# shenwei356/bio

Measured on AMD Instinct MI355X. Metric: Gbases/s hashed (k=21 ntHash + minimizer), higher is better.
Workload: dtype u64

## Files before the change

bio_amd/csrc/biosketch.hip:

```cpp
#include "host_internal.hpp"
#include "kernels_host.hpp"

extern "C" int bsk_abi_version(void) { return BSK_ABI_VERSION; }

extern "C" const char *bsk_err_name(int e) {
    switch (e) {
        case BSK_OK: return "ok";
        case BSK_ERR_INVALID_K: return "ErrInvalidK";
        case BSK_ERR_EMPTY_SEQ: return "ErrEmptySeq";
        case BSK_ERR_SHORT_SEQ: return "ErrShortSeq";
        case BSK_ERR_ILLEGAL_BASE: return "ErrIllegalBase";
        case BSK_ERR_K_TOO_LARGE: return "ErrKTooLarge";
        case BSK_ERR_INVALID_M: return "ErrInvalidM";
        case BSK_ERR_INVALID_SCALE: return "ErrInvalidScale";
        case BSK_ERR_INVALID_S: return "ErrInvalidS";
        case BSK_ERR_INVALID_W: return "ErrInvalidW";
        case BSK_ERR_BUF_NIL: return "ErrBufNil";
        case BSK_ERR_BUF_NOT_EMPTY: return "ErrBufNotEmpty";
        case BSK_ERR_ARG: return "bad argument";
        case BSK_ERR_NOMEM: return "out of memory";
        case BSK_ERR_DEVICE: return "device error";
        case BSK_ERR_UNSUPPORTED: return "unsupported";
        case BSK_ERR_NO_DEVICE: return "no gfx950 device";
        case BSK_ERR_IO: return "fastx: cannot open or read the file";
// ... 138 lines not shown

template <class LenOf>
static void collect_odd(bsk_batch *b, u64 n, LenOf len) {
    delete b->odd;
    b->odd = nullptr;
    b->modal_bucket = -1;
    if (!b->hist || n >= (1ULL << 32)) return;
    int mb = 0;
    for (int i = 1; i < LenHist::NB; ++i)
        if (b->hist->cnt[i] > b->hist->cnt[mb]) mb = i;
    const u64 others = n - b->hist->cnt[mb];
    if (others == 0 || others > n / 20) return;
    auto *v = new (std::nothrow) std::vector<u64>();
    if (!v) return;
    v->reserve((size_t)others);
    for (u64 r = 0; r < n; ++r) {
        const u64 L = len(r);
        if (LenHist::bucket(L) != mb) v->push_back((r << 32) | L);
    }
    b->odd = v;
    b->modal_bucket = mb;
}
static void upload_odd(bsk_ctx *ctx, bsk_batch *b) {
    (void)hipFree(b->d_odd);
    b->d_odd = nullptr;
    if (!b->odd || b->odd->size() < 65536) return;
    if (hipMalloc(&b->d_odd, b->odd->size() * sizeof(u64)) != hipSuccess) {
        (void)hipGetLastError();
        b->d_odd = nullptr;
        return;
    }
    if (hipMemcpyAsync(b->d_odd, b->odd->data(), b->odd->size() * sizeof(u64), hipMemcpyHostToDevice, ctx->stream) != hipSuccess) {
        (void)hipGetLastError();
        (void)hipFree(b->d_odd);
        b->d_odd = nullptr;
    }
}

u64 pad_words(u32 maxlen) { return (u64)maxlen / 16 + kMaxPrefetchWords + 1; }
u32 env_u32(const char *name, u32 dflt) {
    const char *v = getenv(name);
    return v && *v ? (u32)strtoul(v, nullptr, 10) : dflt;
}
u32 min_tile_min(const bsk_ctx *ctx) { return ctx->opt.tile_min ? ctx->opt.tile_min : std::min<u32>(64u, 16u * (BSK_NT_FAST_WORDS - 2)); }
void BskOpts::load() {
    auto on = [](const char *n) { return getenv(n) != nullptr; };
    force_generic = on("BSK_FORCE_GENERIC");
    no_mixed = on("BSK_NO_MIXED");
    no_dense = on("BSK_NO_DENSE");
    no_pk = on("BSK_NO_PK");
    no_ring = on("BSK_NO_RING");
    no_pkd = on("BSK_NO_PKD");
    no_side_early = on("BSK_NO_SIDE_EARLY");
    no_side_dense = on("BSK_NO_SIDE_DENSE");
    no_bin = on("BSK_NO_BIN");
    no_bin_early = on("BSK_NO_BIN_EARLY");
    compact = on("BSK_COMPACT");
    ring = on("BSK_RING");
    ring_max = env_u32("BSK_RING_MAX", 0);
    ring_sel10 = env_u32("BSK_RING_SEL10", 0);
    bin_min = env_u32("BSK_BIN_MIN", 1024);
    no_class = on("BSK_NO_CLASS");
    syn_sel = on("BSK_SYN_SEL");
    class_min = env_u32("BSK_CLASS_MIN", 16384);
    class_force = on("BSK_CLASS_FORCE");
    class_view = on("BSK_CLASS_VIEW");
    no_syn_pf = on("BSK_NO_SYN_PF");
    pf_density = env_u32("BSK_PF_DENSITY", 0);
    no_syn_long = on("BSK_NO_SYN_LONG");
    syn_margin = (int)env_u32("BSK_SYN_MARGIN", (u32)PlannerTable::syn_margin_rows + 64) - 64;
    no_tiles = on("BSK_NO_TILES");
    no_spare = on("BSK_NO_SPARE");
    no_tile_cache = on("BSK_NO_TILE_CACHE");
    tile_dense = on("BSK_TILE_DENSE");
    no_tile_defer = on("BSK_NO_TILE_DEFER");
    no_group_gather = on("BSK_NO_GROUP_GATHER");
    timing = on("BSK_TIMING");
    no_fused_translate = on("BSK_NO_FUSED_TRANSLATE");
    sets_no_small = on("BSK_SETS_NO_SMALL");
    wpr = env_u32("BSK_WPR", 0);
    seg = env_u32("BSK_SEG", 0);
    dense_min = env_u32("BSK_DENSE_MIN", (u32)PlannerTable::dense_min);
    waves_per_cu = env_u32("BSK_WAVES_PER_CU", 0);
    tile_min = env_u32("BSK_TILE_MIN", 0);
    tile_pos = env_u32("BSK_TILE_POS", 0);
    test_overflow = env_u32("BSK_TEST_OVERFLOW", 0);
}
extern "C" int bsk_build_has_experiments(void) {
#ifdef BSK_EXPERIMENTS
    return 1;
#else
    return 0;
#endif
}
extern "C" int bsk_ctx_reload_options(bsk_ctx *ctx) {
    if (!ctx) return BSK_ERR_ARG;
    ctx->opt.load();
    if (ctx->side) ctx->side->opt = ctx->opt;
    return BSK_OK;
}
bsk_ctx *side_ctx(bsk_ctx *ctx) {
    if (!ctx->side) {
        bsk_ctx *s = nullptr;
        if (bsk_ctx_create(ctx->device, &s) != BSK_OK) return nullptr;
        if (hipEventCreateWithFlags(&ctx->ev_side_done, hipEventDisableTiming) != hipSuccess || hipEventCreateWithFlags(&ctx->ev_adopted, hipEventDisableTiming) != hipSuccess ||
            hipEventCreateWithFlags(&ctx->ev_mix0, hipEventDisableTiming) != hipSuccess || hipEventCreateWithFlags(&ctx->ev_mix1, hipEventDisableTiming) != hipSuccess ||
            hipEventCreateWithFlags(&ctx->ev_tiled, hipEventDisableTiming) != hipSuccess) {
            bsk_ctx_destroy(s);
            return nullptr;
        }
        ctx->side = s;
    }
    ctx->side->opt = ctx->opt;
    return ctx->side;
}

static int batch_from_ascii_impl(bsk_ctx *ctx, const uint8_t *bytes, const uint64_t *offsets, uint64_t n, int alphabet, bsk_batch *donor,
                                 bsk_batch **out) {
    if (!ctx || !out || (!offsets && n) || (n && !bytes && offsets[n] > 0)) return fail_arg(ctx, "bsk_batch_from_ascii: null argument");
    if (alphabet < BSK_ALPHA_DNA || alphabet > BSK_ALPHA_UNLIMIT) return fail_arg(ctx, "bad alphabet");
    const int pairs = alphabet == BSK_ALPHA_PROTEIN ? BSK_ALPHA_DNA : alphabet;
    if (alphabet != BSK_ALPHA_PROTEIN) alphabet = BSK_ALPHA_DNA;
    *out = nullptr;
    HIPCHK(ctx, hipSetDevice(ctx->device));
    if (donor && !donor->ascii && donor->spare_ascii) {
        donor->ascii = donor->spare_ascii;
        donor->aoff = donor->spare_aoff;
        donor->spare_ascii = nullptr;
        donor->spare_aoff = nullptr;
    }
    auto take = [&](void **dst, size_t *cap_dst, size_t need, void **src, size_t *cap_src) -> hipError_t {
        if (donor && src && *src && *cap_src >= need) {
            *dst = *src;
            *cap_dst = *cap_src;
            *src = nullptr;
            *cap_src = 0;
            return hipSuccess;
        }
        const size_t want = donor ? need + need / 8 + 256 : need;
        const hipError_t e = hipMalloc(dst, want ? want : 1);
        if (e == hipSuccess) *cap_dst = want;
        return e;
    };
    struct DonorGuard {
        bsk_batch *d;
        ~DonorGuard() { if (d) bsk_batch_destroy(d); }
    } donor_guard{donor};
    bsk_batch *b = new (std::nothrow) bsk_batch();
    if (!b) return BSK_ERR_NOMEM;
    b->ctx = ctx;
    b->alphabet = alphabet;
    b->pairs = pairs;
    b->n = n;
    if (donor) {
        std::swap(b->bdesc, donor->bdesc);
        std::swap(b->c_bdesc, donor->c_bdesc);
        std::swap(b->bflags, donor->bflags);
        std::swap(b->c_bflags, donor->c_bflags);
    }
    const u64 nbytes = n ? offsets[n] : 0;
    b->n_bases = nbytes;
    u32 maxlen = 0;
    bool uniform = true;
    for (u64 r = 0; r < n; ++r) {
        if (offsets[r + 1] < offsets[r]) {
            delete b;
// ... 996 lines not shown
```

bio_amd/csrc/host_types.hpp:

```cpp
#pragma once
#include <hip/hip_runtime.h>

#include <cstdio>
#include <string>
#include <vector>

#include "biosketch.h"
#include "device_common.hpp"

struct BskOpts {
    bool force_generic = false, no_mixed = false, no_dense = false, no_pk = false, no_ring = false, no_pkd = false, no_side_early = false, no_side_dense = false, ring = false, no_bin = false, no_bin_early = false, compact = false, no_spare = false, no_tiles = false, no_tile_cache = false, no_tile_defer = false, tile_dense = false, no_group_gather = false, timing = false,
         no_fused_translate = false, sets_no_small = false;
    int syn_margin = 2;
    u32 test_overflow = 0;
    bool no_syn_long = false;
    u32 pf_density = 0;
    bool no_syn_pf = false;
    bool syn_sel = false;
    bool no_class = false;
    u32 class_min = 16384;
    bool class_view = false;
    bool class_force = false;
    u32 wpr = 0, seg = 0, dense_min = 21 , ring_max = 0, ring_sel10 = 0 , bin_min = 1024, waves_per_cu = 0, tile_min = 0, tile_pos = 0;
    void load();
};

struct bsk_ctx {
    BskOpts opt;
    int device = 0;
    int cus = 0;
    hipStream_t stream = nullptr;
    std::string err;
    u32 *d_ticket = nullptr;
    u64 *d_total = nullptr;
    u64 *d_lookback = nullptr;
    size_t lookback_cap = 0;
    u64 *d_ring_h = nullptr;
    u32 *d_ring_p = nullptr;
    size_t ring_cap = 0;
    u64 *h_pinned = nullptr;
    u8 *d_lut = nullptr;
    int lut_table = 0;
    void *tmp[32] = {};
    size_t tmp_cap[32] = {};
    u64 *h_refs = nullptr;
    size_t h_refs_cap = 0;
    struct bsk_result *tile_res = nullptr;
    static constexpr int SPARE_SLOTS = 8;
    struct Spare {
        void *p = nullptr;
        size_t bytes = 0;
    } spare[SPARE_SLOTS];
    size_t spare_bytes = 0, spare_limit = 0;
    void *comm = nullptr;
    int comm_rank = 0, comm_world = 0;
    u64 *d_comm = nullptr;
    bsk_ctx *side = nullptr;
    hipEvent_t ev_side_done = nullptr, ev_adopted = nullptr, ev_mix0 = nullptr, ev_mix1 = nullptr, ev_tiled = nullptr;
    bool adopted_recorded = false;
    struct ClassSet *cls = nullptr;
    bool no_side_fast = false;
    struct bsk_result *cls_owner = nullptr;
    u64 sel_need = 0;
    bool no_syn_pk = false;
    bool no_prot_fast = false;
    bool defer = false;
    bool tile_sync = false;
    bool tile_async = false;
    bool tile_was_async = false;
    bool in_resize = false;
    int cls_round = 0;
    bool part_grow = false;
    bool no_dense = false;
};

struct LenHist {
    static constexpr int NB = 160;
    u64 cnt[NB] = {}, bases[NB] = {};
    u32 hi[NB] = {};
    u32 lo[NB];
    LenHist() {
        for (int i = 0; i < NB; ++i) lo[i] = 0xffffffffu;
    }
    static int bucket(u64 L) {
        if (L < 1024) return (int)(L >> 4);
        const int lg = 63 - __builtin_clzll(L);
        return 64 + 4 * (lg - 10) + (int)((L >> (lg - 2)) & 3);
    }
    void add(u64 L) {
        const int i = bucket(L);
        cnt[i]++;
        bases[i] += L;
        if ((u32)L > hi[i]) hi[i] = (u32)L;
        if ((u32)L < lo[i]) lo[i] = (u32)L;
    }
};

struct bsk_batch {
    bsk_ctx *ctx = nullptr;
    int alphabet = BSK_ALPHA_DNA;
    int pairs = BSK_ALPHA_DNA;
    u64 n = 0, n_bases = 0, n_words = 0, n_nonacgt = 0;
    u32 maxlen = 0;
    u32 side_maxlen = 0;
    u32 uniform_len = 0;
    u32 *words = nullptr;
// ... 85 lines not shown
```

bio_amd/csrc/kernels_pk.hpp:

```cpp
#pragma once
#include <utility>

#include "kernels_fast.hpp"

namespace bsk {

template <int... Is, class F>
__device__ __forceinline__ void pk_unroll_impl(std::integer_sequence<int, Is...>, F &&f) {
    (f(std::integral_constant<int, Is>{}), ...);
}
template <int N, class F>
__device__ __forceinline__ void pk_unroll(F &&f) {
    pk_unroll_impl(std::make_integer_sequence<int, N>{}, f);
}

#ifndef BSK_PK_ROWS
#define BSK_PK_ROWS 58
#endif
struct PkLds {
    static constexpr int PR = BSK_PK_ROWS;
    static constexpr int ROW = 33;
    static constexpr int TAB = 0;
    static constexpr int TAB2 = 320;
    static constexpr int NHEADS = (32 * (PR - 1)) / 64 + 2;
    static constexpr int HEADS = 0;
    static constexpr int CTAB = 256;
    static constexpr int SH = 768;
    static constexpr int SP = SH + (PR + 1) * ROW * 8;
    static constexpr int TOTAL = (SP + (PR + 1) * ROW * 2 + 15) & ~15;
    static_assert(NHEADS * 8 <= CTAB && CTAB + 512 <= SH && TAB2 + 256 <= SH && TOTAL <= 20480, "PkLds");
};

struct PkTabs {
    u32x4 row;
    u32 at;
    __device__ __forceinline__ void init(int k, int lane, u32 tab = (u32)PkLds::TAB, u32 tab2 = (u32)PkLds::TAB2) {
        row = (u32x4){0, 0, 0, 0};
        at = 0xffffffffu;
        if (lane < 20) {
            const unsigned out = (unsigned)lane >> 2, in = (unsigned)lane & 3u;
            u64 f = seed_fwd_code(in);
            u64 r = rol64(seed_rev_code(in), (unsigned)(k - 1));
            if (out < 4) {
                f ^= rol64(seed_fwd_code(out), (unsigned)k);
                r ^= ror64(seed_rev_code(out), 1);
            }
            row = (u32x4){(u32)f, (u32)(f >> 32), (u32)r, (u32)(r >> 32)};
            at = tab + (u32)lane * 16u;
        } else if (lane >= 32 && lane < 48) {
            const unsigned c0 = (unsigned)lane & 3u, c1 = ((unsigned)lane >> 2) & 3u;
            const u64 f = rol64(seed_fwd_code(c0), 1) ^ seed_fwd_code(c1);
            const u64 r = ror64(rol64(seed_rev_code(c0), (unsigned)(k - 1)), 1) ^ rol64(seed_rev_code(c1), (unsigned)(k - 1));
            row = (u32x4){(u32)f, (u32)(f >> 32), (u32)r, (u32)(r >> 32)};
            at = tab2 + (u32)(lane - 32) * 16u;
        }
    }
    __device__ __forceinline__ void write(LDSQ char *ldsq) const {
        if (at != 0xffffffffu) *reinterpret_cast<LDSQ u32x4 *>(ldsq + at) = row;
        wave_sync_lds();
    }
};

template <int W>
struct PkCfg {
    static constexpr int XC = W > 12 ? 4 : W;
};

#define PKNW 16
typedef u32 u32x16 __attribute__((ext_vector_type(16)));
struct PkWords {
    u32x4 a, b, c, d;
};
__device__ __forceinline__ PkWords pk_load_words(const u32 *p) {
    PkWords r;
    asm volatile("global_load_dwordx4 %0, %4, off\n\tglobal_load_dwordx4 %1, %4, off offset:16\n\t"
                 "global_load_dwordx4 %2, %4, off offset:32\n\tglobal_load_dwordx4 %3, %4, off offset:48"
                 : "=&v"(r.a), "=&v"(r.b), "=&v"(r.c), "=&v"(r.d)
                 : "v"(p));
    return r;
}
__device__ __forceinline__ u64 pk_load_u64(const u64 *p) {
    u64 r;
    asm volatile("global_load_dwordx2 %0, %1, off" : "=&v"(r) : "v"(p));
    return r;
}
__device__ __forceinline__ void pk_wait_loads(u64 &d0, u64 &d1) { asm volatile("s_waitcnt vmcnt(0)" : "+v"(d0), "+v"(d1)::"memory"); }
__device__ __forceinline__ void pk_wait_loads(PkWords &p) { asm volatile("s_waitcnt vmcnt(0)" : "+v"(p.a), "+v"(p.b), "+v"(p.c), "+v"(p.d)::"memory"); }
__device__ __forceinline__ void pk_ticket_async(u32 *ticket, u32 &t) {
    u64 ex;
    asm volatile("s_mov_b64 %1, exec\n\ts_mov_b64 exec, 1\n\tglobal_atomic_add %0, %2, %3, off sc0\n\ts_mov_b64 exec, %1"
                 : "+v"(t), "=&s"(ex)
                 : "v"(ticket), "v"(1u)
                 : "memory");
}
__device__ __forceinline__ void pk_wait_loads(PkWords &p, u64 &d0, u32 &f, u32 &t) {
    asm volatile("s_waitcnt vmcnt(0)" : "+v"(p.a), "+v"(p.b), "+v"(p.c), "+v"(p.d), "+v"(d0), "+v"(f), "+v"(t)::"memory");
}
__device__ __forceinline__ u32 pk_load_u8(const u8 *p) {
    u32 r;
    asm volatile("global_load_ubyte %0, %1, off" : "=&v"(r) : "v"(p));
    return r;
}
template <int W, bool LONG, class LY_ = PkLds, bool RINGM = false, bool SELM = false>
struct PkMin {
    typedef LY_ LY;
    const u32 *__restrict__ w;
    LDSQ char *lds;
    int k, lane;
    u32 nk;
    u32 fl, fh_, rl, rh_;
    u32 S[W];
    u64 H[W];
    u32 SB[W];
    u32 P, bm, tmin;
    u32 nsel;
    u32 slot, spare;
    u32 glo, gspan;
    u32 c8000;
    int sstep;
    u32 send;
    u32 in_lo, in_hi, out_lo, out_hi;
    u32x4 pw;
    u32x16 wr;
    static constexpr bool POS2 = !RINGM && !SELM;
    u32 i2;

    __device__ __forceinline__ void set_words(const PkWords &p) {
        wr = (u32x16){p.a.x, p.a.y, p.a.z, p.a.w, p.b.x, p.b.y, p.b.z, p.b.w, p.c.x, p.c.y, p.c.z, p.c.w, p.d.x, p.d.y, p.d.z, p.d.w};
    }
    __device__ __forceinline__ void word2(u32 i, u32 &lo, u32 &hi) const {
        const u32 iu = (u32)__builtin_amdgcn_readfirstlane((int)i);
        if (!LONG || iu + 1 < (u32)PKNW) {
            lo = wr[iu], hi = wr[iu + 1];
        } else {
            lo = w[iu], hi = w[iu + 1];
        }
    }
    __device__ __forceinline__ u32 word(u32 i) const {
        const u32 iu = (u32)__builtin_amdgcn_readfirstlane((int)i);
        if constexpr (RINGM) {
            if (iu < 4u) return iu == 0 ? pw.x : iu == 1 ? pw.y : iu == 2 ? pw.z : pw.w;
            return w[iu];
        }
        if (!LONG || iu < (u32)PKNW) return wr[iu];
        return w[iu];
    }
    __device__ __forceinline__ void load_block_words(u32 i0) {
        const u32 t0 = i0 + (u32)k - 1, p0 = i0 - 1;
        in_lo = w[t0 >> 4];
        in_hi = w[(t0 >> 4) + 1];
        out_lo = w[p0 >> 4];
        out_hi = w[(p0 >> 4) + 1];
// ... 119 lines not shown
            const u32 nv = (u32)(left < 0 ? 0 : left > W ? W : left);
            vb = (1u << nv) - 1u;
        }
        pk_unroll<W>([&](auto oc) {
            constexpr int o = decltype(oc)::value;
            if (XC < W && o && o % XC == 0 && o + XC < W) {
                __builtin_amdgcn_sched_barrier(0);
                fetch(o + XC);
            }
            roll(xs[o]);
            if (!FIRST) this->template emit<PB + o, o>(pbase);
            const lmask rev = lt64(rl, rh_, fl, fh_);
            const u32 hl = sel(rev, rl, fl), hh = sel(rev, rh_, fh_);
            if constexpr (POS2) {
                lmask co;
                asm("v_addc_co_u32_e64 %0, %1, %2, %3, %4" : "=v"(SB[o]), "=s"(co) : "n"(2 * o), "v"(i2), "s"(rev));
            } else {
                asm("v_cndmask_b32_e64 %0, 0, %1, %2" : "=v"(SB[o]) : "v"(c8000), "s"(rev));
            }
            H[o] = ((u64)hh << 32) | hl;
            u32 pk;
            asm("v_and_or_b32 %0, %1, %2, %3" : "=v"(pk) : "v"(hh), "s"(0xffffffe0u), "n"(CB + o));
            if (o == 0) {
                P = pk;
            } else {
#ifndef PK_NOTIE
                const u32 d = pk ^ P;
                tmin = tmin < d ? tmin : d;
#endif
                P = P < pk ? P : pk;
            }
            if (!FIRST || o == W - 1) {
                u32 m = P;
                if constexpr (o != W - 1) {
#ifndef PK_NOTIE
                    const u32 d = P ^ S[o + 1];
                    tmin = tmin < d ? tmin : d;
#endif
                    m = P < S[o + 1] ? P : S[o + 1];
                }
                u32 one = 1u;
                if (FIRST) one = okbit;
                else if (RAG) one = (vb >> o) & 1u;
                bm |= one << (m & 31u);
            }
            S[o] = pk;
        });
        if (suffix) {
#pragma unroll
            for (int q = W - 2; q >= 0; --q) {
#ifndef PK_NOTIE
                const u32 d = S[q] ^ S[q + 1];
                tmin = tmin < d ? tmin : d;
#endif
                S[q] = S[q] < S[q + 1] ? S[q] : S[q + 1];
            }
        }
        if constexpr (SELM) {
            if (!FIRST) {
                const u32 wsel = (bm >> PB) & ((1u << W) - 1u);
                *reinterpret_cast<LDSQ u32 *>(lds + LY::MASK + (i0 / (u32)W - 1u) * 256u + (u32)lane * 4u) = wsel;
                nsel += (u32)__builtin_popcount(wsel);
            }
        }
        if (!FIRST) bm &= PAR ? 0xffff0000u : 0x0000ffffu;
    }

    template <int PAR>
    __device__ __forceinline__ void drain(u32 i0) {
        if constexpr (SELM) {
            const u32 wsel = (bm >> (PAR * 16)) & ((1u << W) - 1u);
            *reinterpret_cast<LDSQ u32 *>(lds + LY::MASK + (i0 / (u32)W) * 256u + (u32)lane * 4u) = wsel;
            nsel += (u32)__builtin_popcount(wsel);
            return;
        }
        const u32 pbase = (u32)__builtin_amdgcn_readfirstlane((int)i0);
        guard();
        pk_unroll<W>([&](auto oc) {
            constexpr int o = decltype(oc)::value;
            this->template emit<PAR * 16 + o, o>(pbase);
        });
    }

    __device__ __forceinline__ void begin(u32 slot0, int step, u32 col8) {
        fl = fh_ = rl = rh_ = 0;
        bm = 0;
        nsel = 0;
        c8000 = 0x8000u;
        asm volatile("" : "+v"(c8000));
        tmin = 0xffffffffu;
        slot = slot0;
        sstep = step;
        if constexpr (RINGM) {
            (void)col8;
            spare = glo = gspan = 0;
            send = (u32)(LY::ROWS * LY::ROW * 8) + (u32)lane * 8u;
        } else {
            spare = (u32)(LY::PR * LY::ROW * 8) + col8;
            send = 0;
            constexpr u32 RB = (u32)(LY::ROW * 8);
            glo = step < 0 ? col8 + (u32)(W - 1) * RB : col8;
            gspan = (u32)(LY::PR - W) * RB + (step < 0 ? 0u : RB);
        }
        if constexpr (RINGM) load_block0_words();
        for (int t0 = 0; t0 < k - 1; t0 += 16) {
            const u32 word = this->word((u32)t0 >> 4);
            const int nb = (k - 1 - t0) < 16 ? (k - 1 - t0) : 16;
            int j = 0;
            for (; j + 8 <= nb; j += 8) {
                const u32 sub = word >> (2 * j);
                const u32x4 x0 = *reinterpret_cast<LDSQ const u32x4 *>(lds + LY::TAB2 + ((sub & 0xf) << 4));
                const u32x4 x1 = *reinterpret_cast<LDSQ const u32x4 *>(lds + LY::TAB2 + (sub & 0xf0));
                const u32x4 x2 = *reinterpret_cast<LDSQ const u32x4 *>(lds + LY::TAB2 + ((sub & 0xf00) >> 4));
                const u32x4 x3 = *reinterpret_cast<LDSQ const u32x4 *>(lds + LY::TAB2 + ((sub & 0xf000) >> 8));
                roll2(x0);
                roll2(x1);
                roll2(x2);
                roll2(x3);
            }
            for (; j + 2 <= nb; j += 2) roll2(*reinterpret_cast<LDSQ const u32x4 *>(lds + LY::TAB2 + (((word >> (2 * j)) & 0xf) << 4)));
            for (; j < nb; ++j) roll(*reinterpret_cast<LDSQ const u32x4 *>(lds + LY::TAB + 256 + (((word >> (2 * j)) & 3) << 4)));
        }
    }

    __device__ __forceinline__ void run(u32 nk_max, bool ok, u32 nk_min, u32 slot0, int step, u32 col8) {
        begin(slot0, step, col8);
        block<true, false, 0>(0, ok ? 1u : 0u, nk_max > (u32)W);
        u32 i0 = W;
        int last_par = 0;
        for (;;) {
            if (i0 >= nk_max) break;
            {
                const bool more = i0 + W < nk_max;
                if (i0 + W <= nk_min) block<false, false, 1>(i0, 1u, more);
                else block<false, true, 1>(i0, 1u, more);
            }
            i0 += W;
            last_par = 1;
            if (i0 >= nk_max) break;
            {
                const bool more = i0 + W < nk_max;
                if (i0 + W <= nk_min) block<false, false, 0>(i0, 1u, more);
                else block<false, true, 0>(i0, 1u, more);
            }
            i0 += W;
            last_par = 0;
        }
        if (last_par) drain<1>(i0 - W);
        else drain<0>(i0 - W);
    }
};

template <int U, class LY = PkLds, bool POS2 = false>
__device__ __forceinline__ void pk_copyout(char *lds, int lane, u32 cnt, u32 excl, u32 T, u64 base, const KArgs &a) {
    constexpr int NH = LY::NHEADS;
    u64 *s_heads = reinterpret_cast<u64 *>(lds + LY::HEADS);
    u64 *s_tab64 = reinterpret_cast<u64 *>(lds + LY::CTAB);
    const u64 nzmask = __builtin_amdgcn_ballot_w64(cnt > 0);
    if (lane < NH) s_heads[lane] = 0;
    wave_sync_lds();
    if (cnt > 0) {
        constexpr int RB = LY::ROW * 8;
        const int col8 = (lane & 31) * 8;
        const int S = lane < 32 ? RB : -RB;
        const int A = lane < 32 ? col8 - (int)excl * RB : col8 + ((int)(LY::PR - 1) + (int)excl) * RB;
        const u32 rk = __builtin_amdgcn_mbcnt_hi((u32)(nzmask >> 32), __builtin_amdgcn_mbcnt_lo((u32)nzmask, 0));
        s_tab64[rk] = ((u64)(u32)S << 32) | (u32)A;
        if (excl) atomicOr(&s_heads[(excl - 1u) >> 6], 1ULL << ((excl - 1u) & 63u));
    }
    wave_sync_lds();
    const u64 hw = lane < NH ? s_heads[lane] : 0ULL;
    const u32 hw_lo = (u32)hw, hw_hi = (u32)(hw >> 32);
    u32 heads_before = 0;
    const char *sh = lds + LY::SH, *sp = lds + LY::SP;
    u64 *const gh = a.hash + base;
    u32 *const gp = a.pos + base;
    auto trip = [&](u32 t0, auto check) {
        constexpr bool CHECK = decltype(check)::value;
        u32 rank[U];
#pragma unroll
        for (int j = 0; j < U; ++j) {
            const u32 c = (t0 >> 6) + j;
            const u32 mlo = (u32)__builtin_amdgcn_readlane((int)hw_lo, (int)c), mhi = (u32)__builtin_amdgcn_readlane((int)hw_hi, (int)c);
            rank[j] = (__builtin_amdgcn_mbcnt_hi(mhi, __builtin_amdgcn_mbcnt_lo(mlo, 0u)) << 3) + (heads_before << 3);
            heads_before += (u32)__builtin_popcountll(((u64)mhi << 32) | mlo);
        }
        u64 ent[U];
#pragma unroll
        for (int j = 0; j < U; ++j) ent[j] = *reinterpret_cast<const u64 *>(reinterpret_cast<const char *>(s_tab64) + rank[j]);
        if constexpr (U == 8) {
            __builtin_amdgcn_sched_barrier(0);
            asm volatile("" ::"v"(ent[0]), "v"(ent[1]), "v"(ent[2]), "v"(ent[3]), "v"(ent[4]), "v"(ent[5]), "v"(ent[6]), "v"(ent[7]));
            __builtin_amdgcn_sched_barrier(0);
        }
        u64 hv[U];
        u32 pv[U];
#pragma unroll
        for (int j = 0; j < U; ++j) {
            const u32 t = t0 + 64 * j + lane;
            const int off = __mul24((int)t, (int)(u32)(ent[j] >> 32)) + (int)(u32)ent[j];
            const u32 so = (!CHECK || t < T) ? (u32)off : 0u;
            hv[j] = *reinterpret_cast<const u64 *>(sh + so);
            if constexpr (POS2) pv[j] = *reinterpret_cast<const u16 *>(sp + (so >> 2));
            else pv[j] = (u32)(int)*reinterpret_cast<const short *>(sp + (so >> 2));
        }
        if constexpr (U == 8) {
            __builtin_amdgcn_sched_barrier(0);
            asm volatile("" ::"v"(hv[0]), "v"(hv[1]), "v"(hv[2]), "v"(hv[3]), "v"(hv[4]), "v"(hv[5]), "v"(hv[6]), "v"(hv[7]), "v"(pv[0]), "v"(pv[1]),
                         "v"(pv[2]), "v"(pv[3]), "v"(pv[4]), "v"(pv[5]), "v"(pv[6]), "v"(pv[7]));
            __builtin_amdgcn_sched_barrier(0);
        }
#pragma unroll
        for (int j = 0; j < U; ++j) {
            const u32 t = t0 + 64 * j + lane;
#ifdef PK_NOSTORE
            asm volatile("" ::"v"(hv[j]), "v"(pv[j]));
#else
            if (!CHECK || t < T) {
#ifndef PK_NOHASHST
                __builtin_nontemporal_store(hv[j], &gh[t]);
#else
                asm volatile("" ::"v"(hv[j]));
#endif
#ifndef PK_NOPOSST
                __builtin_nontemporal_store(POS2 ? __builtin_amdgcn_alignbit(pv[j], pv[j], 1) : pv[j] & 0x80007fffu, &gp[t]);
#else
                asm volatile("" ::"v"(pv[j]));
#endif
            }
#endif
        }
    };
    u32 t0 = 0;
    for (; t0 + 64 * U <= T; t0 += 64 * U) trip(t0, std::false_type{});
    if (t0 < T) trip(t0, std::true_type{});
    wave_sync_lds();
}

#ifndef PK_TICKET
#define PK_TICKET 8u
#endif
template <int W, bool LONG>
__global__ __launch_bounds__(64, 2) void k_minimizer_pk(KArgs a) {
    typedef PkLds LY;
    __shared__ __attribute__((aligned(16))) char lds[LY::TOTAL];
    LDSQ char *const ldsq = (LDSQ char *)lds;
    const int lane = lane_id();
    PkTabs tabs;
    tabs.init(a.k, lane);
#ifdef PK_STAGGER
    for (u32 i = (((blockIdx.x * 2654435761u) >> 24) * (u32)PK_STAGGER) >> 8; i; --i) __builtin_amdgcn_s_sleep(32);
#endif
    const u64 slab = (u64)64 * BSK_FAST_CAP;
    const u32 col8 = (u32)(lane & 31) * 8u;
    constexpr u32 RB = (u32)(LY::ROW * 8);
    const u32 top = (u32)(LY::PR - 1) * RB + col8;
    u64 d_n1 = 0, d_cur = 0;
    PkWords pw_cur = {{0, 0, 0, 0}, {0, 0, 0, 0}, {0, 0, 0, 0}, {0, 0, 0, 0}};
    bool have = false;
    const u32 lseg = a.fixcap / a.list_grid;
    u32 lcur = 0;
    const u32 tku = a.tk ? a.tk : PK_TICKET;
    const bool ahead = tku >= 3u;
    u32 tv = 0;
    u32 nt = ~0u;
    for (u32 unit = next_ticket(a.ticket, lane) * tku, uend = unit + tku; unit < a.nunits; ++unit, ({
             if (unit == uend) {
                 unit = ahead ? nt : next_ticket(a.ticket, lane) * tku;
                 uend = unit + tku;
             }
         })) {
        const u64 r = (u64)unit * 64 + lane;
        const u64 u2 = (!ahead || unit + 2u < uend) ? (u64)unit + 2u : (u64)nt + (unit + 2u - uend);
        const bool nxt = unit + 1 != uend ? unit + 1 < a.nunits : ahead && nt < a.nunits;
        const bool ask = ahead && unit + 3u == uend;
        const u64 rmax = a.n - 1;
        if (!have) {
            d_cur = pk_load_u64(a.desc + (r < rmax ? r : rmax));
            d_n1 = pk_load_u64(a.desc + (r + 64 < rmax ? r + 64 : rmax));
            pk_wait_loads(d_cur, d_n1);
            pw_cur = pk_load_words(a.words + (d_cur >> 24));
            pk_wait_loads(pw_cur);
        }
        PkWords pw_n1 = pk_load_words(a.words + (d_n1 >> 24));
        const u64 r2 = u2 * 64 + lane;
        u64 d_n2 = pk_load_u64(a.desc + (r2 < rmax ? r2 : rmax));
        u32 rfl = pk_load_u8(a.rflags ? a.rflags + (r < rmax ? r : rmax) : reinterpret_cast<const u8 *>(a.desc));
        if (ask) pk_ticket_async(a.ticket, tv);
        const u64 d = d_cur;
        const PkWords pw = pw_cur;
        const u64 off = d >> 24, L = desc_len(a, d);
        const u64 ro = out_index(a, r, d);
        const bool ok = r < a.n && L >= (u64)a.circ_ext && (L - (u64)a.circ_ext) + 1 >= (u64)a.k + (u64)W;
        const u32 nk = ok ? (u32)(L - a.k + 1) : 0u;
        const u32 nk_max = wave_max_u32(nk);
        const u32 nk_min = ~wave_max_u32(~(ok ? nk : 0xffffffffu));
        u32 cnt = 0, tmin_lane = 0xffffffffu;
        if (nk_max) {
            tabs.write(ldsq);
            PkMin<W, LONG> pm;
            pm.w = a.words + off;
            pm.set_words(pw);
            pm.lds = ldsq;
            pm.k = a.k;
            pm.lane = lane;
            pm.nk = nk;
            const u32 spare = (u32)LY::PR * RB + col8;
            pm.run(nk_max, ok, nk_min, !ok ? spare : lane < 32 ? col8 : top, !ok ? 0 : lane < 32 ? (int)RB : -(int)RB, col8);
            if (ok) cnt = (lane < 32 ? pm.slot - col8 : top - pm.slot) / RB;
            tmin_lane = pm.tmin;
        }
        pk_wait_loads(pw_n1, d_n2, rfl, tv);
        if (ask) nt = (u32)__builtin_amdgcn_readfirstlane((int)tv) * tku;
        d_cur = d_n1;
        pw_cur = pw_n1;
        d_n1 = d_n2;
        have = nxt;
        const u32 cnt_pair = cnt + (u32)__builtin_amdgcn_ds_bpermute((lane ^ 32) * 4, (int)cnt);
        u64 bad = __builtin_amdgcn_ballot_w64(cnt_pair >= (u32)LY::PR);
        u64 tied = __builtin_amdgcn_ballot_w64(ok && tmin_lane < 32u);
#if defined(PK_NOSTAGE) || defined(PK_NOTIE) || defined(PK_NOTAB) || defined(PK_NOCOPY) || defined(PK_NOSTORE) || defined(PK_NOFB)
        bad = 0;
        tied = 0;
#endif
        const u64 redo = bad | tied;
        if (redo) {
            list_append(a, a.rlist, lseg, lcur, redo, lane, r);
            if ((redo >> lane) & 1) cnt = 0;
        }
        const u32 incl = wave_incl_scan_u32(cnt, lane);
        const u32 excl = incl - cnt;
        const u32 T = wave_bcast_u32(incl, 63);
        const u64 base = (u64)unit * slab;
#ifndef PK_NOCOPY
#ifndef PK_CU
#define PK_CU 8
#endif
        if (T) pk_copyout<PK_CU, LY, PkMin<W, LONG>::POS2>(lds, lane, cnt, excl, T, base, a);
#endif
        if (r < a.n) {
            if (!((redo >> lane) & 1)) a.refs[ro] = ((base + excl) << 24) | cnt;
            u8 sbyte = ok ? BSK_ST_OK : BSK_ST_SHORT;
            if (ok && a.rflags) sbyte |= (u8)rfl;
            a.status[ro] = sbyte;
        }
    }
    list_close(a.rlist, lseg, lcur, lane);
}

#ifdef BSK_IMPL_PK
#ifndef BSK_PK_WS
#define BSK_PK_WS(X) X(2) X(3) X(4) X(5) X(6) X(7) X(8) X(9) X(10) X(11) X(12) X(13)
#endif
bool pk_minimizer_supported(int w) { return w >= 2 && w <= 13; }
u32 pk_minimizer_short_bases() { return 16u * (PKNW - 1); }
int pk_minimizer_blocks_per_cu(int w) {
    int nb = 0;
    hipError_t e = hipErrorInvalidValue;
    switch (w) {
#define X(WW) \
    case WW: e = hipOccupancyMaxActiveBlocksPerMultiprocessor(&nb, k_minimizer_pk<WW, false>, 64, 0); break;
        BSK_PK_WS(X)
#undef X
        default: break;
    }
    if (e != hipSuccess || nb < 1) {
        (void)hipGetLastError();
        nb = 1;
    }
    return nb;
}
void pk_minimizer_list_launch(int w, int grid, hipStream_t stream, const KArgs &a) {
    switch (w) {
#define X(WW) \
    case WW: hipLaunchKernelGGL((k_minimizer_dense<WW, true>), dim3(grid), dim3(64), 0, stream, a); break;
        BSK_PK_WS(X)
#undef X
        default: break;
    }
}
void pk_minimizer_launch(int w, bool long_reads, int grid, hipStream_t stream, const KArgs &a) {
    switch (w) {
#define X(WW)                                                                                               \
    case WW:                                                                                                \
        if (long_reads) {                                                                                   \
            hipLaunchKernelGGL((k_minimizer_pk<WW, true>), dim3(grid), dim3(64), 0, stream, a);             \
        } else {                                                                                            \
            hipLaunchKernelGGL((k_minimizer_pk<WW, false>), dim3(grid), dim3(64), 0, stream, a);            \
        }                                                                                                   \
        hipLaunchKernelGGL((k_minimizer_dense<WW, true>), dim3(grid), dim3(64), 0, stream, a);              \
        break;
        BSK_PK_WS(X)
#undef X
        default: break;
    }
// ... 5 lines not shown
```

bio_amd/csrc/planner.hip:

```cpp
#include "host_internal.hpp"
#include "kernels_host.hpp"

int validate(const bsk_params *p, int alphabet) {
    switch (p->kind) {
        case BSK_NTHASH:
            if (p->k < 1) return BSK_ERR_INVALID_K;
            break;
        case BSK_KMER:
            if (p->k < 1) return BSK_ERR_INVALID_K;
            if (p->k > 32) return BSK_ERR_K_TOO_LARGE;
            break;
        case BSK_SIMHASH:
            if (p->k < 1) return BSK_ERR_INVALID_K;
            if (p->k >= 65535) return BSK_ERR_K_TOO_LARGE;
            if (p->m < 4 || p->m > p->k) return BSK_ERR_INVALID_M;
            if (p->scale < 1 || p->scale > p->k - p->m + 1) return BSK_ERR_INVALID_SCALE;
            if (p->k - p->m + 1 > 32767) return BSK_ERR_UNSUPPORTED;
            break;
        case BSK_MINIMIZER:
            if (p->k < 1) return BSK_ERR_INVALID_K;
            if (p->w < 1) return BSK_ERR_INVALID_W;
            break;
        case BSK_SYNCMER:
            if (p->k < 1) return BSK_ERR_INVALID_K;
// ... 340 lines not shown
            pl.slab = true;
            pl.slab_unit = (u64)64 * BSK_SYN_CAP;
            pl.slab_total = (u64)pl.nunits * pl.slab_unit;
            pl.bin_gran = bin_gran_for(ctx, b, p->k - p->s);
            per_cu = fast_syncmer_blocks_per_cu(pl.fast_w);
        } else {
            pl.which = use_ascii ? K_SYN_A : K_SYN_P;
            per_cu = use_ascii ? occ(OCC_SYN_A) : occ(OCC_SYN_P);
            pl.ring_w = (u32)std::max(1, 2 * (p->k - p->s));
        }
    } else if (p->kind == BSK_KMER) {
        if (!use_ascii && p->canonical > 0 && b->maxlen + (u32)(p->circular ? p->k : 0) <= 16u * (BSK_NT_FAST_WORDS - 2) &&
            !ctx->opt.force_generic) {
            pl.which = K_NT_FAST;
            pl.compact = stream_compact_ok(ctx, b, p);
            per_cu = occ(OCC_NT_FAST2);
#ifdef BSK_EXPERIMENTS
            if (pl.compact) per_cu = occ(OCC_NT_FAST2C);
#endif
        } else if (!use_ascii && p->canonical <= 0 && !p->circular && b->maxlen <= 16u * (BSK_NT_FAST_WORDS - 2) && !ctx->opt.force_generic) {
            pl.which = K_NT_FAST;
            per_cu = occ(p->canonical < 0 ? OCC_NT_FAST4 : OCC_NT_FAST3);
        } else {
            pl.which = use_ascii ? K_KMER_A : K_KMER_P;
            per_cu = use_ascii ? occ(OCC_KMER_A) : occ(OCC_KMER_P);
        }
    } else if (p->kind == BSK_SIMHASH) {
        const int nh = p->k - p->m + 1;
        if (!use_ascii && nh <= 63 && b->maxlen + (u32)(p->circular ? p->k : 0) <= 16u * (BSK_NT_FAST_WORDS - 2) &&
            !ctx->opt.force_generic) {
            pl.which = K_SIM_FAST;
            pl.fast_w = nh <= 31 ? 5 : 6;
            const u32 ext_len = b->maxlen + (u32)(p->circular ? p->k : 0);
            pl.fast_k = ext_len <= 16u * (BSK_SIM_SHORT_WORDS - 2) ? 1 : ext_len <= 16u * (BSK_SIM_MID_WORDS - 2) ? 2 : 0;
            if (pl.fast_k == 1) per_cu = nh <= 31 ? occ(OCC_SIMF_5S) : occ(OCC_SIMF_6S);
            else if (pl.fast_k == 2) per_cu = nh <= 31 ? occ(OCC_SIMF_5M) : occ(OCC_SIMF_6M);
            else per_cu = nh <= 31 ? occ(OCC_SIMF_5) : occ(OCC_SIMF_6);
        } else {
            pl.which = use_ascii ? K_SIM_A : K_SIM_P;
            per_cu = use_ascii ? occ(OCC_SIM_A) : occ(OCC_SIM_P);
            pl.ring_w = (u32)nh;
        }
    } else if (p->kind == BSK_PROT_HASH) {
        if (b->alphabet == BSK_ALPHA_DNA) {
            pl.which = K_PROT_HASH_FAST;
            pl.fused_dna = true;
            pl.fast_k = p->k;
            per_cu = fast_prot_hash_dna_blocks_per_cu(p->k);
        } else if (fast_prot_hash_supported(p->k) && !ctx->opt.force_generic) {
            pl.which = K_PROT_HASH_FAST;
            pl.fast_k = p->k;
            per_cu = fast_prot_hash_blocks_per_cu(p->k);
        } else {
            pl.which = K_PROT_HASH;
            per_cu = occ(OCC_PROT_HASH);
        }
    } else if (p->kind == BSK_PROT_MINIMIZER) {
        const u32 plen = b->alphabet == BSK_ALPHA_DNA ? (u32)translated_len(b->maxlen, 1) : b->maxlen;
        if (b->alphabet == BSK_ALPHA_DNA && ctx->no_prot_fast) return BSK_REPLAN_UNFUSED;
        if (b->alphabet == BSK_ALPHA_DNA || (fast_prot_supported(p->w, p->k) && b->maxlen < 65536u && b->maxlen >= (u32)(p->k + p->w) && !ctx->opt.force_generic &&
            !ctx->no_prot_fast && slab_budget_ok(b, (u64)b->maxlen))) {
            pl.which = K_PROT_MIN_FAST;
            pl.fused_dna = b->alphabet == BSK_ALPHA_DNA;
            pl.fast_w = p->w;
            pl.fast_k = p->k;
            pl.slab = true;
            const u64 nwin = plen >= (u32)(p->k + p->w) ? (u64)plen - p->k - p->w + 2 : 1;
            pl.slab_read = std::min<u64>(nwin, (u64)(nwin * PlannerTable::slab_sel_num / (p->w + 1.0)) + PlannerTable::slab_sel_pad);
            pl.slab_read = (pl.slab_read + 15) & ~(u64)15;
            pl.slab_unit = 64 * pl.slab_read;
            pl.slab_total = (u64)pl.nunits * pl.slab_unit;
            per_cu = fast_prot_blocks_per_cu(p->w, p->k);
        } else {
            pl.which = K_PROT_MIN;
            per_cu = occ(OCC_PROT_MIN);
            pl.ring_w = (u32)p->w;
        }
    } else {
        ctx->err = "unknown kind";
        return BSK_ERR_ARG;
    }
    if (ctx->opt.waves_per_cu) per_cu = (int)ctx->opt.waves_per_cu;
    pl.grid = (int)std::max<u64>(1, std::min<u64>((u64)ctx->cus * per_cu, pl.nunits));
    pl.ring_entries = (size_t)pl.grid * pl.ring_w * 64;
    return BSK_OK;
}


void plan_name(const Plan &pl, const bsk_params *p, bool tiled, int cus, bsk_result *res) {
    char b[80];
    switch (pl.which) {
        case K_MIN_GEN_P: snprintf(b, sizeof b, "k_minimizer_generic<0>"); break;
        case K_MIN_GEN_A: snprintf(b, sizeof b, "k_minimizer_generic<1>"); break;
        case K_NT_P: snprintf(b, sizeof b, "k_nthash_stream<0>"); break;
        case K_NT_A: snprintf(b, sizeof b, "k_nthash_stream<1>"); break;
        case K_MIN_FAST: snprintf(b, sizeof b, "k_minimizer_fast<%d,%d,true>", pl.fast_w, BSK_FAST_CAP); break;
        case K_MIN_PK: snprintf(b, sizeof b, "k_minimizer_pk<%d,%s>", pl.fast_w, pl.fast_k ? "true" : "false"); break;
        case K_MIN_RING: snprintf(b, sizeof b, "k_minimizer_ring<%d,%s>", pl.fast_w, pl.fast_k ? "true" : "false"); break;
        case K_MIN_DENSE: snprintf(b, sizeof b, "k_minimizer_dense<%d>", pl.fast_w); break;
        case K_MIN_PKD: snprintf(b, sizeof b, "k_minimizer_pkd<%d>", pl.fast_w); break;
        case K_MIN_SEG: snprintf(b, sizeof b, "k_minimizer_seg<%d>", pl.fast_w); break;
        case K_MIN_WPR: snprintf(b, sizeof b, "k_minimizer_wpr<%d>", pl.fast_w); break;
        case K_NT_FAST: snprintf(b, sizeof b, pl.compact ? "k_nthash_fast<%d,true>" : "k_nthash_fast<%d>", p->kind == BSK_KMER ? (p->canonical > 0 ? 2 : p->canonical < 0 ? 4 : 3) : p->canonical ? 1 : 0); break;
        case K_SYN_P: snprintf(b, sizeof b, "k_syncmer<0>"); break;
        case K_SYN_A: snprintf(b, sizeof b, "k_syncmer<1>"); break;
        case K_KMER_P: snprintf(b, sizeof b, "k_kmer<0>"); break;
        case K_KMER_A: snprintf(b, sizeof b, "k_kmer<1>"); break;
        case K_SIM_P: snprintf(b, sizeof b, "k_simhash<0>"); break;
        case K_SIM_A: snprintf(b, sizeof b, "k_simhash<1>"); break;
        case K_PROT_HASH: snprintf(b, sizeof b, "k_prot_hash"); break;
        case K_PROT_MIN: snprintf(b, sizeof b, "k_prot_minimizer"); break;
        case K_SYN_FAST: snprintf(b, sizeof b, "k_syncmer_fast<%d>", pl.fast_w); break;
        case K_SYN_PK: snprintf(b, sizeof b, pl.syn_fused ? (pl.syn_long ? "k_syncmer_pfl<%d>" : "k_syncmer_pf<%d>") : pl.syn_long ? "k_syncmer_pkl<%d>" : "k_syncmer_pk<%d>", pl.fast_w); break;
        case K_SYN_SEL: snprintf(b, sizeof b, "k_syncmer_sel<%d> + k_syncmer_emit", pl.fast_w); break;
        case K_PROT_MIN_FAST: snprintf(b, sizeof b, "k_prot_minimizer_fast<%d,%d,%s>", pl.fast_w, pl.fast_k, pl.fused_dna ? "true" : "false"); break;
        case K_PROT_HASH_FAST: snprintf(b, sizeof b, "k_prot_hash_fast<%d,%s>", pl.fast_k, pl.fused_dna ? "true" : "false"); break;
        case K_SIM_FAST:
            snprintf(b, sizeof b, "k_simhash_fast<%d,%d>", pl.fast_w, pl.fast_k == 1 ? BSK_SIM_SHORT_WORDS : pl.fast_k == 2 ? BSK_SIM_MID_WORDS : BSK_NT_FAST_WORDS);
            break;
        default: snprintf(b, sizeof b, "?"); break;
    }
    snprintf(res->plan, sizeof res->plan, "%s%s%s%s", b, pl.bin_gran ? " (length-binned units)" : "", pl.mixed ? " + ASCII side launch" : "", tiled ? " (over tiles)" : "");
    res->plan_grid = pl.grid;
    res->plan_per_cu = cus > 0 ? (pl.grid + cus - 1) / cus : 0;
}

u64 syn_pk_fixcap(u64 n, int grid) { return std::max<u64>((u64)grid * 1024, (n / 4 + (u64)grid) / (u64)grid * (u64)grid); }
```

Baseline: 1237.

## Overlap next-row k-mer warmup with drain in packed minimizer kernel

Splits the packed minimizer's run into reset, warmup, blocks and drain phases. While draining the final window block, it rolls the first k-1 bases of the next row (using the already-prefetched next words) into the hash state, so the next iteration can skip its serial warmup. The wait for the next row's loads moves before the drain so those words are available. This adds register pressure (16 u32x4 LDS lookups held live) and applies only when k-1 fits in 32 bases. It also adds a BSK_GRID_MAX env knob that caps the grid size, which is off by default.

```diff
diff --git a/bio_amd/csrc/biosketch.hip b/bio_amd/csrc/biosketch.hip
--- a/bio_amd/csrc/biosketch.hip
+++ b/bio_amd/csrc/biosketch.hip
@@ -244,6 +244,7 @@
     seg = env_u32("BSK_SEG", 0);
     dense_min = env_u32("BSK_DENSE_MIN", (u32)PlannerTable::dense_min);
     waves_per_cu = env_u32("BSK_WAVES_PER_CU", 0);
+    grid_max = env_u32("BSK_GRID_MAX", 0);
     tile_min = env_u32("BSK_TILE_MIN", 0);
     tile_pos = env_u32("BSK_TILE_POS", 0);
     test_overflow = env_u32("BSK_TEST_OVERFLOW", 0);
diff --git a/bio_amd/csrc/host_types.hpp b/bio_amd/csrc/host_types.hpp
--- a/bio_amd/csrc/host_types.hpp
+++ b/bio_amd/csrc/host_types.hpp
@@ -21,7 +21,7 @@
     u32 class_min = 16384;
     bool class_view = false;
     bool class_force = false;
-    u32 wpr = 0, seg = 0, dense_min = 21 , ring_max = 0, ring_sel10 = 0 , bin_min = 1024, waves_per_cu = 0, tile_min = 0, tile_pos = 0;
+    u32 wpr = 0, seg = 0, dense_min = 21 , ring_max = 0, ring_sel10 = 0 , bin_min = 1024, waves_per_cu = 0, grid_max = 0 , tile_min = 0, tile_pos = 0;
     void load();
 };
 
diff --git a/bio_amd/csrc/kernels_pk.hpp b/bio_amd/csrc/kernels_pk.hpp
--- a/bio_amd/csrc/kernels_pk.hpp
+++ b/bio_amd/csrc/kernels_pk.hpp
@@ -68,6 +68,9 @@
 
 #define PKNW 16
 typedef u32 u32x16 __attribute__((ext_vector_type(16)));
+struct PkWarm {
+    u32 fl, fh, rl, rh;
+};
 struct PkWords {
     u32x4 a, b, c, d;
 };
@@ -353,7 +356,55 @@
         });
     }
 
+    static constexpr int WARM_SLOTS = 16, WARM_BASES = 2 * WARM_SLOTS;
+    template <int BYTE>
+    static __device__ __forceinline__ u32 nib16(u32 src) {
+        u32 a;
+        if constexpr (BYTE == 0) asm("v_and_b32_sdwa %0, %1, %2 dst_sel:DWORD dst_unused:UNUSED_PAD src0_sel:BYTE_0 src1_sel:DWORD" : "=v"(a) : "v"(src), "s"(0xF0u));
+        else if constexpr (BYTE == 1) asm("v_and_b32_sdwa %0, %1, %2 dst_sel:DWORD dst_unused:UNUSED_PAD src0_sel:BYTE_1 src1_sel:DWORD" : "=v"(a) : "v"(src), "s"(0xF0u));
+        else if constexpr (BYTE == 2) asm("v_and_b32_sdwa %0, %1, %2 dst_sel:DWORD dst_unused:UNUSED_PAD src0_sel:BYTE_2 src1_sel:DWORD" : "=v"(a) : "v"(src), "s"(0xF0u));
+        else asm("v_and_b32_sdwa %0, %1, %2 dst_sel:DWORD dst_unused:UNUSED_PAD src0_sel:BYTE_3 src1_sel:DWORD" : "=v"(a) : "v"(src), "s"(0xF0u));
+        return a;
+    }
+    template <int PAR>
+    __device__ __forceinline__ void drain_warm(u32 i0, u32 w0, u32 w1) {
+        static_assert(!RINGM && !SELM, "drain_warm");
+        const u32 pbase = (u32)__builtin_amdgcn_readfirstlane((int)i0);
+        guard();
+        fl = fh_ = rl = rh_ = 0;
+        const int nb = k - 1 <= WARM_BASES ? k - 1 : 0;
+        const int n2 = nb >> 1;
+        u32x4 xr[WARM_SLOTS];
+        const u32 w04 = w0 << 4, w14 = w1 << 4;
+        pk_unroll<WARM_SLOTS / 4>([&](auto gc) {
+            constexpr int g = decltype(gc)::value;
+            if (4 * g < n2) {
+                const u32 lo = g < 2 ? w04 : w14, hi = g < 2 ? w0 : w1;
+                constexpr int B = 2 * (g & 1);
+                xr[4 * g + 0] = *reinterpret_cast<LDSQ const u32x4 *>(lds + LY::TAB2 + nib16<B>(lo));
+                xr[4 * g + 1] = *reinterpret_cast<LDSQ const u32x4 *>(lds + LY::TAB2 + nib16<B>(hi));
+                xr[4 * g + 2] = *reinterpret_cast<LDSQ const u32x4 *>(lds + LY::TAB2 + nib16<B + 1>(lo));
+                xr[4 * g + 3] = *reinterpret_cast<LDSQ const u32x4 *>(lds + LY::TAB2 + nib16<B + 1>(hi));
+            }
+        });
+        const u32 c1 = (u32)((((u64)w1 << 32) | w0) >> ((4 * n2) & 63)) & 3u;
+        const u32x4 x1 = *reinterpret_cast<LDSQ const u32x4 *>(lds + LY::TAB + 256 + (c1 << 4));
+        pk_unroll<W>([&](auto oc) {
+            constexpr int o = decltype(oc)::value;
+            this->template emit<PAR * 16 + o, o>(pbase);
+            pk_unroll<(o + 1) * WARM_SLOTS / W - o * WARM_SLOTS / W>([&](auto jc) {
+                constexpr int j = o * WARM_SLOTS / W + decltype(jc)::value;
+                if (j < n2) roll2(xr[j]);
+            });
+        });
+        if (nb & 1) roll(x1);
+    }
+
     __device__ __forceinline__ void begin(u32 slot0, int step, u32 col8) {
+        reset(slot0, step, col8);
+        warmup();
+    }
+    __device__ __forceinline__ void reset(u32 slot0, int step, u32 col8) {
         fl = fh_ = rl = rh_ = 0;
         bm = 0;
         nsel = 0;
@@ -373,6 +424,8 @@
             glo = step < 0 ? col8 + (u32)(W - 1) * RB : col8;
             gspan = (u32)(LY::PR - W) * RB + (step < 0 ? 0u : RB);
         }
+    }
+    __device__ __forceinline__ void warmup() {
         if constexpr (RINGM) load_block0_words();
         for (int t0 = 0; t0 < k - 1; t0 += 16) {
             const u32 word = this->word((u32)t0 >> 4);
@@ -396,6 +449,11 @@
 
     __device__ __forceinline__ void run(u32 nk_max, bool ok, u32 nk_min, u32 slot0, int step, u32 col8) {
         begin(slot0, step, col8);
+        u32 il;
+        if (blocks(nk_max, ok, nk_min, il)) drain<1>(il);
+        else drain<0>(il);
+    }
+    __device__ __forceinline__ int blocks(u32 nk_max, bool ok, u32 nk_min, u32 &il) {
         block<true, false, 0>(0, ok ? 1u : 0u, nk_max > (u32)W);
         u32 i0 = W;
         int last_par = 0;
@@ -417,8 +475,8 @@
             i0 += W;
             last_par = 0;
         }
-        if (last_par) drain<1>(i0 - W);
-        else drain<0>(i0 - W);
+        il = i0 - W;
+        return last_par;
     }
 };
 
@@ -529,6 +587,8 @@
     u64 d_n1 = 0, d_cur = 0;
     PkWords pw_cur = {{0, 0, 0, 0}, {0, 0, 0, 0}, {0, 0, 0, 0}, {0, 0, 0, 0}};
     bool have = false;
+    PkWarm wm = {0, 0, 0, 0};
+    bool warm = false;
     const u32 lseg = a.fixcap / a.list_grid;
     u32 lcur = 0;
     const u32 tku = a.tk ? a.tk : PK_TICKET;
@@ -567,9 +627,11 @@
         const u32 nk_max = wave_max_u32(nk);
         const u32 nk_min = ~wave_max_u32(~(ok ? nk : 0xffffffffu));
         u32 cnt = 0, tmin_lane = 0xffffffffu;
+        PkMin<W, LONG> pm;
+        u32 il = 0;
+        int lpar = 0;
         if (nk_max) {
             tabs.write(ldsq);
-            PkMin<W, LONG> pm;
             pm.w = a.words + off;
             pm.set_words(pw);
             pm.lds = ldsq;
@@ -577,11 +639,21 @@
             pm.lane = lane;
             pm.nk = nk;
             const u32 spare = (u32)LY::PR * RB + col8;
-            pm.run(nk_max, ok, nk_min, !ok ? spare : lane < 32 ? col8 : top, !ok ? 0 : lane < 32 ? (int)RB : -(int)RB, col8);
+            pm.reset(!ok ? spare : lane < 32 ? col8 : top, !ok ? 0 : lane < 32 ? (int)RB : -(int)RB, col8);
+            if (warm) pm.fl = wm.fl, pm.fh_ = wm.fh, pm.rl = wm.rl, pm.rh_ = wm.rh;
+            else pm.warmup();
+            lpar = pm.blocks(nk_max, ok, nk_min, il);
+        }
+        pk_wait_loads(pw_n1, d_n2, rfl, tv);
+        warm = false;
+        if (nk_max) {
+            if (lpar) pm.template drain_warm<1>(il, pw_n1.a.x, pw_n1.a.y);
+            else pm.template drain_warm<0>(il, pw_n1.a.x, pw_n1.a.y);
+            wm.fl = pm.fl, wm.fh = pm.fh_, wm.rl = pm.rl, wm.rh = pm.rh_;
+            warm = nxt && a.k - 1 <= PkMin<W, LONG>::WARM_BASES;
             if (ok) cnt = (lane < 32 ? pm.slot - col8 : top - pm.slot) / RB;
             tmin_lane = pm.tmin;
         }
-        pk_wait_loads(pw_n1, d_n2, rfl, tv);
         if (ask) nt = (u32)__builtin_amdgcn_readfirstlane((int)tv) * tku;
         d_cur = d_n1;
         pw_cur = pw_n1;
diff --git a/bio_amd/csrc/planner.hip b/bio_amd/csrc/planner.hip
--- a/bio_amd/csrc/planner.hip
+++ b/bio_amd/csrc/planner.hip
@@ -446,6 +446,7 @@
     }
     if (ctx->opt.waves_per_cu) per_cu = (int)ctx->opt.waves_per_cu;
     pl.grid = (int)std::max<u64>(1, std::min<u64>((u64)ctx->cus * per_cu, pl.nunits));
+    if (ctx->opt.grid_max) pl.grid = (int)std::min<u64>((u64)pl.grid, ctx->opt.grid_max);
     pl.ring_entries = (size_t)pl.grid * pl.ring_w * 64;
     return BSK_OK;
 }
```

After: 1141. -7.8%, worse.
